# zhaobinglei/REGNet_for_3D_Grasping

Hardware: AMD Instinct MI355X
Metric: scenes/sec (25 600-pt ScoreNet+GRN fwd) (higher is better)
Workload: dtype f32; 1 GPU; configs[2]: ScoreNet+GraspRegionNet+RefineNet forward, 25600-pt synthetic scenes, batch=8 per GPU, eval; points=25600, batch_per_gpu=8, global_batch=8, parallelism=scene-sharded x1 (no data-path collective), sampling_group_batches=8, sampling_lookahead_batches=32, distinct_batches=8, region_head=synthetic.calibrate_region_head on batch 0, geometry_pending_at_enqueue=4, hip_graphs=False

## Files before the change

### include/regnet_hip.h

```cpp
#ifndef REGNET_HIP_H_
#define REGNET_HIP_H_

#include <stdint.h>

#ifdef __cplusplus
extern "C" {
#endif

#define REGNET_OK 0
#define REGNET_ERR_SHAPE (-1)
#define REGNET_ERR_NULL (-2)
#define REGNET_ERR_UNSUPPORTED (-3)

int regnet_abi_version(void);
const char* regnet_build_info(void);
const char* regnet_strerror(int code);

int regnet_fps_f32(const float* xyz, int64_t sb, int64_t sc, int64_t sn, int64_t B, int64_t N,
                   int64_t M, int64_t* index, float* workspace, void* stream);
int64_t regnet_fps_workspace_bytes(int64_t B, int64_t N, int64_t M);
int regnet_fps_chain_f32(const float* xyz, int64_t sb, int64_t sc, int64_t sn, int64_t B, int64_t N, int64_t M,
                         int64_t* index, float* workspace, const int32_t* prefix_ok, int32_t* first_tie, void* stream);
int64_t regnet_fps_status_offset_bytes(int64_t B, int64_t N, int64_t M);
int regnet_fps_plan(int64_t B, int64_t N, int64_t M, int64_t* plan);
// ... 179 lines not shown
                                int64_t label_ld, int64_t C, float radius, float score_thre, int64_t m, float* final_grasp,
                                uint8_t* flags, float* terms, float* dreg, void* stream);

int regnet_gripper_frame_f32(const float* grasp, int64_t ld, int64_t n, float* centre, float* rot, void* stream);
int regnet_crop_pick(const int32_t* cand, int64_t G, const int64_t* pos, int64_t R, const uint8_t* valid,
                     const int64_t* group_index, int64_t gi_stride, int64_t n, int64_t* index, int64_t* index_inall,
                     void* stream);

int regnet_resample_groups_f32(const float* pc, int64_t pb, int64_t pn, int64_t C, const int32_t* cand, int64_t cap,
                               const int64_t* pos, int64_t B, int64_t Nc, int64_t G, int64_t N, int32_t* out_of_range,
                               int64_t* index, float* points, void* stream);

int64_t regnet_normals_workspace_bytes(int64_t N);
int regnet_estimate_normals_f32(const float* xyz, int64_t N, double radius, int64_t max_nn, double cam_x, double cam_y,
                                double cam_z, float* normals, int32_t* count, void* workspace, void* stream);

int64_t regnet_bn_workspace_bytes(int64_t C);
int regnet_bn_relu_train_fwd_f32(const float* x, int64_t B, int64_t C, int64_t L, const float* gamma, const float* beta,
                                 float eps, float momentum, float* running_mean, float* running_var, int relu,
                                 int64_t pool_group, float* y, int32_t* pool_index, float* save_mean, float* save_invstd,
                                 void* workspace, void* stream);
int regnet_bn_relu_train_bwd_f32(const float* x, const float* y, const float* dy, const int32_t* pool_index, int64_t B,
                                 int64_t C, int64_t L, const float* gamma, const float* beta, const float* save_mean,
                                 const float* save_invstd, int relu, int64_t pool_group, float* dx, float* dgamma,
                                 float* dbeta, void* workspace, void* stream);

int regnet_bn_train_stats_f32(const float* x, int64_t B, int64_t C, int64_t L, const float* gamma, const float* beta, float eps,
                              float momentum, float* running_mean, float* running_var, float* save_mean, float* save_invstd,
                              float* scale, float* shift, void* workspace, void* stream);
int regnet_bn_relu_train_fwd_from_sums_f32(const float* x, int64_t B, int64_t C, int64_t L, const float* gamma, const float* beta,
                                           float eps, float momentum, float* running_mean, float* running_var, int relu,
                                           int64_t pool_group, float* y, int32_t* pool_index, float* save_mean,
                                           float* save_invstd, void* workspace, void* stream);
int regnet_bn_train_stats_from_sums_f32(int64_t B, int64_t C, int64_t L, const float* gamma, const float* beta, float eps,
                                        float momentum, float* running_mean, float* running_var, float* save_mean,
                                        float* save_invstd, float* scale, float* shift, void* workspace, void* stream);

int regnet_sa_premul_layer_f32(const float* U, int64_t ldu, const float* V, int64_t ldv, int64_t C1,
                               const int64_t* nbr, int64_t B, int64_t Nsrc, int64_t M, int64_t group,
                               const float* W, int64_t Kpad, const float* scale, const float* shift,
                               float* C, int64_t ldc, int64_t N, int relu, int pool_group, void* stream);

int regnet_interp_concat_f32(const float* sparse, int64_t sb, int64_t sn, int64_t Cs,
                             const int64_t* idx, const float* dist2, float eps, const float* dense,
                             int64_t db, int64_t dn, int64_t dc, int64_t Cd, int64_t B, int64_t Nd,
                             float* out, int64_t ldo, int64_t Cout, void* stream);

int regnet_interp_affine_f32(const float* ys, int64_t sb, int64_t sn, const int64_t* idx,
                             const float* dist2, float eps, const float* yd, int64_t ldd,
                             const float* dense_small, int64_t db, int64_t dn, int64_t dc,
                             int64_t Cd_small, const float* Wd4, const float* scale, const float* shift,
                             int relu, int64_t B, int64_t Nd, int64_t C, float* out, int64_t ldo,
                             void* stream);

int regnet_score_head_f32(const float* x, int64_t ldx, int64_t C, const float* w, float bias,
                          float bn_scale, float bn_shift, float* score, int64_t P, void* stream);

int64_t regnet_sa_premul_chain_stream_floats(void);
int regnet_sa_premul_chain_f32(const float* U, int64_t ldu, const float* V, int64_t ldv, const int64_t* nbr, int64_t B,
                               int64_t Nsrc, int64_t M, const float* stream_w, int64_t n_stages, const float* affine,
                               int64_t affine_floats, int relu3, float* out, int64_t ldo, int32_t* ticket,
                               void* stream);

int64_t regnet_sa3_premul_chain_stream_floats(void);
int regnet_sa3_premul_chain_f32(const float* U, int64_t ldu, const float* V, int64_t ldv, const int64_t* nbr, int64_t B,
                                int64_t Nsrc, int64_t M, const float* stream_w, int64_t n_stages, const float* affine,
                                int64_t affine_floats, int relu3, float* out, int64_t ldo, int32_t* ticket,
                                void* stream);

int64_t regnet_fp_head_chain_stream_floats(void);
int64_t regnet_fp_head_chain_blocks(int64_t P);
int regnet_fp_head_chain_interp_f32(const float* Ys, int64_t ys_sb, int64_t ys_sn, const int64_t* idx,
                                    const float* dist2, float eps, const float* dense_small, int64_t db, int64_t dn,
                                    int64_t dc, int64_t Cd_small, const float* tables, int64_t B, int64_t Nd,
                                    const float* stream_w, int64_t n_stages, const float* affine, int64_t affine_floats,
                                    const float* wscore, float score_bias, float score_bn_scale, float score_bn_shift,
                                    float* F, int64_t ldf, float* score, int32_t* ticket, int64_t block_first,
                                    int64_t block_count, void* stream);
int regnet_fp_head_chain_f32(const float* X, int64_t ldx, const float* stream_w, int64_t n_stages,
                             const float* affine, int64_t affine_floats, const float* wscore, float score_bias,
                             float score_bn_scale, float score_bn_shift, float* F, int64_t ldf, float* score,
                             int64_t P, int32_t* ticket, int64_t block_first, int64_t block_count, void* stream);

int regnet_conv1x1_train_supported(int64_t Co, int64_t Ci, int64_t L);
int regnet_conv1x1_fwd_f32(const float* W, const float* X, float* Y, int64_t B, int64_t Co, int64_t Ci, int64_t L,
                           void* stream);
int regnet_conv1x1_dgrad_f32(const float* W, const float* dY, float* dX, int64_t B, int64_t Co, int64_t Ci, int64_t L,
                             void* stream);
int regnet_conv1x1_fwd_stream_f32(const float* W, const float* X, float* Y, int64_t B, int64_t Co, int64_t Ci, int64_t L,
                                  int32_t* ticket, void* stream);
int regnet_conv1x1_dgrad_stream_f32(const float* W, const float* dY, float* dX, int64_t B, int64_t Co, int64_t Ci, int64_t L,
                                    int32_t* ticket, void* stream);
int regnet_conv1x1_fwd_smallci_f32(const float* W, const float* X, float* Y, int64_t B, int64_t Co, int64_t Ci, int64_t L,
                                   void* stream);
int64_t regnet_conv1x1_smallci_stats_workspace_bytes(int64_t B, int64_t Ci, int64_t L);
int regnet_conv1x1_fwd_smallci_stats_f32(const float* W, const float* X, float* Y, int64_t B, int64_t Co, int64_t Ci, int64_t L,
                                         void* workspace, void* sums, void* stream);
int64_t regnet_conv1x1_wgrad_smallci_partials(int64_t B, int64_t Co, int64_t L);
int regnet_conv1x1_wgrad_smallci_f32(const float* dY, const float* X, float* part, int64_t B, int64_t Co, int64_t Ci, int64_t L,
                                     void* stream);
int regnet_conv1x1_smallco_f32(int dir, const float* W, const float* bias, const float* in, float* out, int64_t B, int64_t Co,
                               int64_t Ci, int64_t L, void* stream);
int regnet_conv1x1_stream_reserve_slots(int slots);
int64_t regnet_sa_chain3_split_plane_bytes(int64_t C3);
int regnet_sa_chain3_split_f32(const float* feat, int64_t fb, int64_t fn, int64_t fc, int64_t Cf, const float* xyz, int64_t xb,
                               int64_t xc, int64_t xn, const int64_t* nbr, const int64_t* ctr, const int64_t* count,
// ... 86 lines not shown
```

### regnet_for_3d_grasping_amd/csrc/gemm2.h

```cpp
#pragma once
#include "common.h"

typedef float g2_f32x16 __attribute__((ext_vector_type(16)));

#define G2_BK 16

struct G2Args {
  const float* A; long long lda; int Ka;
  const float* W; int Kpad;
  const float* scale; const float* shift;
  float* C; long long ldc;
  long long P; int N; int relu;
  int tiles_m, tiles_n;
  int main_blocks, tail_tiles, tail_split;
};

__device__ __forceinline__ void g2_glds16(const float* gsrc, unsigned lds_dst) {
  unsigned keep;
  asm volatile("s_mov_b32 %0, m0\n\ts_mov_b32 m0, %2\n\ts_nop 0\n\tglobal_load_lds_dwordx4 %1, off\n\ts_mov_b32 m0, %0"
               : "=&s"(keep) : "v"(gsrc), "s"(lds_dst) : "memory");
}

template <int N> __device__ __forceinline__ void g2_wait_barrier() {
  asm volatile("s_waitcnt vmcnt(%0)\n\ts_barrier" :: "i"(N) : "memory");
}

__device__ __forceinline__ long long g2_xcd_linear(unsigned vblock, long long total) {
  const long long q = total / 8, r = total % 8;
  const long long xcd = vblock % 8, s = vblock / 8;
  return (xcd < r ? xcd * (q + 1) : r * (q + 1) + (xcd - r) * q) + s;
}

template <int ROWS_MAX, int TBN, int WM, int WN, int TM, int STAGES, bool POOL, int SLAB_KT>
__device__ __forceinline__ void g2_tile(const G2Args& p, float* smem, long long row0, int col0) {
  constexpr int NW = WM * WN;
  constexpr int ROWS = WM * TM * 32;
  constexpr int TN = TBN / WN / 32;
  constexpr int STAGE_FLOATS = (ROWS_MAX + TBN) * G2_BK;
  constexpr int GROUPS = (ROWS + TBN) / 16;
  constexpr int L = (GROUPS + NW - 1) / NW;
  static_assert(GROUPS % NW == 0, "every wave issues the same number of LDS-DMA pieces");
  constexpr int D = STAGES - 1;
  const int tid = threadIdx.x, lane = tid & 63;
  const int wave = __builtin_amdgcn_readfirstlane(tid >> 6);
  const int wm = wave / WN, wn = wave % WN;
  const int fr = lane & 31, fh = lane >> 5;

  const float* gp[L];
  unsigned dst[L];
  bool isA[L];
  const int lrow = lane >> 2, lchunk = (lane & 3) ^ ((lane >> 4) & 3);
#pragma unroll
  for (int j = 0; j < L; ++j) {
    const int grp = wave + j * NW;
    const int cr = grp * 16 + lrow;
    isA[j] = grp * 16 < ROWS;
    if (isA[j]) {
      long long r = row0 + cr;
      if (r >= p.P) r = 0;
      gp[j] = p.A + r * p.lda + 4 * lchunk;
    } else {
      gp[j] = p.W + (long long)(col0 + cr - ROWS) * p.Kpad + 4 * lchunk;
    }
    dst[j] = (unsigned)(grp * 16 * G2_BK * 4);
  }
  const unsigned smem_base = (unsigned)(uintptr_t)smem;
  const bool ragged_k = p.Ka < p.Kpad;

#define G2_ISSUE(KT_, STAGE_)                                                                                   \
  _Pragma("unroll") for (int j = 0; j < L; ++j) {                                                                \
    const float* src = gp[j] + (long long)(KT_) * G2_BK;                                                         \
    if (ragged_k && isA[j] && (KT_) * G2_BK + 4 * lchunk >= p.Ka) src = gp[j] - 4 * lchunk;    \
    g2_glds16(src, smem_base + (unsigned)((STAGE_) * STAGE_FLOATS * 4) + dst[j]);                                \
  }

  g2_f32x16 acc[TM][TN];
#pragma unroll
  for (int mi = 0; mi < TM; ++mi)
#pragma unroll
    for (int ni = 0; ni < TN; ++ni)
#pragma unroll
      for (int r = 0; r < 16; ++r) acc[mi][ni][r] = 0.f;

  g2_f32x16 tot[SLAB_KT > 0 ? TM : 1][SLAB_KT > 0 ? TN : 1];
  if constexpr (SLAB_KT > 0) {
#pragma unroll
// ... 33 lines not shown
#define G2_PIN() __builtin_amdgcn_sched_barrier(0)
#else
#define G2_PIN()
#endif
#define G2_COMPUTE(STAGE_)                                                                                        \
  {                                                                                                               \
    const float* st = smem + (STAGE_) * STAGE_FLOATS;                                                             \
    float4 a[2][TM], b[2][TN];        \
    _Pragma("unroll") for (int kk = 0; kk < 2; ++kk) {                                                            \
      _Pragma("unroll") for (int mi = 0; mi < TM; ++mi)                                                           \
        a[kk][mi] = *reinterpret_cast<const float4*>(st + offA[kk] + mi * 32 * G2_BK);                            \
      _Pragma("unroll") for (int ni = 0; ni < TN; ++ni)                                                           \
        b[kk][ni] = *reinterpret_cast<const float4*>(st + offW[kk] + ni * 32 * G2_BK);                            \
    }                                                                                                             \
    G2_PIN();                                                                                                     \
    _Pragma("unroll") for (int kk = 0; kk < 2; ++kk)                                                              \
      _Pragma("unroll") for (int mi = 0; mi < TM; ++mi)                                                           \
        _Pragma("unroll") for (int ni = 0; ni < TN; ++ni) {                                                       \
          acc[mi][ni] = __builtin_amdgcn_mfma_f32_32x32x2f32(a[kk][mi].x, b[kk][ni].x, acc[mi][ni], 0, 0, 0);     \
          acc[mi][ni] = __builtin_amdgcn_mfma_f32_32x32x2f32(a[kk][mi].y, b[kk][ni].y, acc[mi][ni], 0, 0, 0);     \
          acc[mi][ni] = __builtin_amdgcn_mfma_f32_32x32x2f32(a[kk][mi].z, b[kk][ni].z, acc[mi][ni], 0, 0, 0);     \
          acc[mi][ni] = __builtin_amdgcn_mfma_f32_32x32x2f32(a[kk][mi].w, b[kk][ni].w, acc[mi][ni], 0, 0, 0);     \
        }                                                                                                         \
  }
#pragma unroll
  for (int d = 0; d < D; ++d) { G2_ISSUE(d, d) }
  int stage = 0;
  for (int kt = 0; kt < KT - D; ++kt) {
    g2_wait_barrier<(D - 1) * L>();
    int ns = stage + D; if (ns >= STAGES) ns -= STAGES;
    G2_ISSUE(kt + D, ns)
    G2_COMPUTE(stage)
    G2_SLAB()
    if (++stage == STAGES) stage = 0;
  }
#pragma unroll
  for (int d = 0; d < D; ++d) {
    g2_wait_barrier<0>();
    G2_COMPUTE(stage)
    G2_SLAB()
    if (++stage == STAGES) stage = 0;
  }
  if constexpr (SLAB_KT > 0) {
#pragma unroll
    for (int mi = 0; mi < TM; ++mi)
#pragma unroll
      for (int ni = 0; ni < TN; ++ni)
#pragma unroll
        for (int r = 0; r < 16; ++r) acc[mi][ni][r] += tot[mi][ni][r];
  }
#undef G2_SLAB
#undef G2_COMPUTE
#undef G2_ISSUE
#pragma unroll
  for (int ni = 0; ni < TN; ++ni) {
    const int col = col0 + (wn * TN + ni) * 32 + fr;
    const bool col_ok = col < p.N;
    const float s = col_ok ? p.scale[col] : 0.f, t = col_ok ? p.shift[col] : 0.f;
    if (POOL) {
      static_assert(!POOL || TM == 2, "pooling: a wave's 64 rows are one neighbourhood");
      float m = -__builtin_inff();
#pragma unroll
      for (int mi = 0; mi < TM; ++mi)
#pragma unroll
        for (int r = 0; r < 16; ++r) {
          float y = acc[mi][ni][r] * s + t;
          if (p.relu) y = fmaxf(y, 0.f);
          m = fmaxf(m, y);
        }
      m = fmaxf(m, __shfl_xor(m, 32, 64));
      const long long wrow = row0 + wm * 64;
      if (col_ok && fh == 0 && wrow < p.P) p.C[(wrow / 64) * p.ldc + col] = m;
    } else {
      const long long first_row = row0 + wm * TM * 32 + 4 * fh;
      float* cp = p.C + first_row * p.ldc + col;
      const long long ld = p.ldc;
      const bool interior = (row0 + ROWS <= p.P) && (col0 + TBN <= p.N);
      if (interior) {
#pragma unroll
        for (int mi = 0; mi < TM; ++mi)
#pragma unroll
          for (int r = 0; r < 16; ++r) {
            float y = acc[mi][ni][r] * s + t;
            if (p.relu) y = fmaxf(y, 0.f);
            *cp = y;
            cp += ((r & 3) == 3) ? 5 * ld : ld;
          }
      } else {
#pragma unroll
        for (int mi = 0; mi < TM; ++mi)
#pragma unroll
          for (int r = 0; r < 16; ++r) {
            float y = acc[mi][ni][r] * s + t;
            if (p.relu) y = fmaxf(y, 0.f);
            if (col_ok && first_row + mi * 32 + (r & 3) + 8 * (r >> 2) < p.P) *cp = y;
            cp += ((r & 3) == 3) ? 5 * ld : ld;
          }
      }
    }
  }
}

#ifndef G2_SLAB_KT
#define G2_SLAB_KT 8
#endif
template <int TBM, int TBN, int WM, int WN, int WG_PER_CU> struct G2Slab {
  static constexpr int acc_tiles = (TBM / WM / 32) * (TBN / WN / 32);
  static constexpr int kt = (acc_tiles <= 2 || (acc_tiles <= 4 && WG_PER_CU * WM * WN <= 8)) ? G2_SLAB_KT : 0;
};

template <int TBM, int TBN, int WM, int WN, int STAGES, int WG_PER_CU, bool POOL>
__global__ __launch_bounds__(WM * WN * 64, WG_PER_CU * WM * WN / 4)
void gemm2_kernel(const G2Args p) {
  constexpr int SLAB = G2Slab<TBM, TBN, WM, WN, WG_PER_CU>::kt;
  constexpr int TM = TBM / WM / 32;
  __shared__ __attribute__((aligned(1024))) float smem[STAGES * (TBM + TBN) * G2_BK];
  const int bid = blockIdx.x;
  if (bid < p.main_blocks) {
    const long long t = g2_xcd_linear((unsigned)bid, p.main_blocks);
    const int tm = (int)(t / p.tiles_n), tn = (int)(t % p.tiles_n);
    g2_tile<TBM, TBN, WM, WN, TM, STAGES, POOL, SLAB>(p, smem, (long long)tm * TBM, tn * TBN);
  } else if constexpr (!POOL && TM == 2 && ((WM * 32 + TBN) / 16) % (WM * WN) == 0) {
    const int t = (bid - p.main_blocks) / p.tail_split, s = (bid - p.main_blocks) % p.tail_split;
    const long long tile = (long long)p.main_blocks + t;
    const int tm = (int)(tile / p.tiles_n), tn = (int)(tile % p.tiles_n);
    g2_tile<TBM, TBN, WM, WN, 1, STAGES, false, SLAB>(p, smem, (long long)tm * TBM + (long long)s * (TBM / 2), tn * TBN);
  }
}
```

### regnet_for_3d_grasping_amd/csrc/mlp.hip

```cpp
#include <stdlib.h>
#include "common.h"
#include "gemm2.h"

typedef float f32x16 __attribute__((ext_vector_type(16)));

#define BM 128
#define BN 128
#define MLP_THREADS 256
#ifndef MLP_BK
#define MLP_BK 16
#endif
#define BK MLP_BK
#ifndef MLP_ABLATE
#define MLP_ABLATE 0
#endif
#ifndef MLP_TRACE
#define MLP_TRACE 0
#endif
#define LDS_LD (BK + 4)
#define ROWS_PER_PASS (MLP_THREADS / (BK / 4))
#define STAGE_PASSES (BM / ROWS_PER_PASS)
#ifndef MLP_MIN_WAVES
#define MLP_MIN_WAVES (BK == 32 ? 2 : 4)
#endif
// ... 403 lines not shown
};

template <int TBM, int TBN, int WM, int WN, int STAGES, int OCC>
static int plan_gemm2_tile(int tile, long long P, int N, bool pool, G2Plan& pl) {
  pl.tile = tile; pl.tbm = TBM; pl.tbn = TBN; pl.waves = WM * WN; pl.wg_per_cu = OCC;
  pl.slab_kt = G2Slab<TBM, TBN, WM, WN, OCC>::kt;
  pl.tiles_m = (int)((P + TBM - 1) / TBM);
  pl.tiles_n = (N + TBN - 1) / TBN;
  const long long tiles = (long long)pl.tiles_m * pl.tiles_n;
  if (tiles >= (1ll << 30)) return REGNET_ERR_UNSUPPORTED;
  const long long slots = (long long)G2_CUS * OCC;
  long long main_blocks = tiles, tail_tiles = 0;
  constexpr bool can_split = (TBM / WM / 32 == 2) && ((WM * 32 + TBN) / 16) % (WM * WN) == 0;
  if (!pool && can_split && tiles > slots) {
    const long long rem = tiles % slots;
    if (rem > 0 && rem * 2 <= slots) { main_blocks = tiles - rem; tail_tiles = rem; }
  }
  pl.main_blocks = (int)main_blocks; pl.tail_tiles = (int)tail_tiles; pl.tail_split = 2;
  if (pool && TBM / WM != 64) return REGNET_ERR_UNSUPPORTED;
  return REGNET_OK;
}

static int plan_gemm2(long long P, int N, int Kpad, bool pool, G2Plan& pl) {
  static const int force_tile = getenv("REGNET_G2_TILE") ? atoi(getenv("REGNET_G2_TILE")) : -1;
  if (force_tile == 0) return plan_gemm2_tile<G2_TILE_256>(0, P, N, pool, pl);
  if (force_tile == 1) return plan_gemm2_tile<G2_TILE_128>(1, P, N, pool, pl);
  if (force_tile == 2) return plan_gemm2_tile<G2_TILE_64>(2, P, N, pool, pl);
  if (force_tile == 3 && !pool) return plan_gemm2_tile<G2_TILE_128W8>(3, P, N, pool, pl);
  if (force_tile == 8 && !pool) return plan_gemm2_tile<G2_TILE_128S>(8, P, N, pool, pl);
  const long long nt = (N + 127) / 128;
  const long long t256 = ((P + 255) / 256) * nt, t128 = ((P + 127) / 128) * nt;
  if (N > 128 && t256 >= 4 * G2_CUS) return plan_gemm2_tile<G2_TILE_256>(0, P, N, pool, pl);
  static const bool t8 = !(getenv("REGNET_G2_T8") && getenv("REGNET_G2_T8")[0] == '0');
  if (t8 && !pool && G2_SLAB_KT > 0 && Kpad >= 2 * G2_SLAB_KT * G2_BK && t128 >= G2_CUS)
    return plan_gemm2_tile<G2_TILE_128S>(8, P, N, pool, pl);
  if (t128 >= 4 * G2_CUS && (G2_SLAB_KT == 0 || Kpad < 2 * G2_SLAB_KT * G2_BK || pool))
    return plan_gemm2_tile<G2_TILE_128>(1, P, N, pool, pl);
  return plan_gemm2_tile<G2_TILE_64>(2, P, N, pool, pl);
}

template <int TBM, int TBN, int WM, int WN, int STAGES, int OCC>
static int launch_gemm2_tile(const G2Args& g, bool pool, hipStream_t st) {
  const dim3 grid((unsigned)(g.main_blocks + g.tail_split * g.tail_tiles)), block(WM * WN * 64);
  if (pool) {
    if constexpr (TBM / WM == 64) hipLaunchKernelGGL((gemm2_kernel<TBM, TBN, WM, WN, STAGES, OCC, true>), grid, block, 0, st, g);
    else return REGNET_ERR_UNSUPPORTED;
  } else {
    hipLaunchKernelGGL((gemm2_kernel<TBM, TBN, WM, WN, STAGES, OCC, false>), grid, block, 0, st, g);
  }
  REGNET_LAUNCH_CHECK();
  return REGNET_OK;
}

static int launch_gemm2(G2Args g, const G2Plan& pl, bool pool, hipStream_t st) {
  g.tiles_m = pl.tiles_m; g.tiles_n = pl.tiles_n;
  g.main_blocks = pl.main_blocks; g.tail_tiles = pl.tail_tiles; g.tail_split = pl.tail_split;
  switch (pl.tile) {
    case 0: return launch_gemm2_tile<G2_TILE_256>(g, pool, st);
    case 1: return launch_gemm2_tile<G2_TILE_128>(g, pool, st);
    case 2: return launch_gemm2_tile<G2_TILE_64>(g, pool, st);
    case 3: return launch_gemm2_tile<G2_TILE_128W8>(g, pool, st);
    case 8: return launch_gemm2_tile<G2_TILE_128S>(g, pool, st);
  }
  return REGNET_ERR_UNSUPPORTED;
}

struct MlpLayerPlan { bool gemm2; G2Plan g2; long long blocks; };
static int plan_mlp_layer(long long P, long long N, long long Kpad, int pool_group, MlpLayerPlan& pl) {
  pl = MlpLayerPlan{};
  if (P < 0 || N <= 0 || Kpad <= 0 || Kpad % BK) return REGNET_ERR_SHAPE;
  if (pool_group != 0 && (pool_group != 64 || P % 64)) return REGNET_ERR_UNSUPPORTED;
  if (P == 0) return REGNET_OK;
  static const bool use_gemm2 = MLP_USE_GEMM2 && !(getenv("REGNET_GEMM2") && getenv("REGNET_GEMM2")[0] == '0');
  if (use_gemm2 && Kpad >= 2 * G2_BK) {
    pl.gemm2 = true;
    return plan_gemm2(P, (int)N, (int)Kpad, pool_group != 0, pl.g2);
  }
  pl.blocks = ((P + BM - 1) / BM) * ((N + BN - 1) / BN);
  return pl.blocks >= (1ll << 31) ? REGNET_ERR_UNSUPPORTED : REGNET_OK;
}

extern "C" int regnet_mlp_layer_plan(int64_t P, int64_t N, int64_t Kpad, int pool_group, int64_t* plan) {
  if (!plan) return REGNET_ERR_NULL;
  for (int i = 0; i < 8; ++i) plan[i] = 0;
  MlpLayerPlan pl;
  const int rc = plan_mlp_layer(P, N, Kpad, pool_group, pl);
  if (rc != REGNET_OK || P == 0) return rc;
  if (pl.gemm2) {
    const G2Plan& g = pl.g2;
    plan[0] = g.tbm; plan[1] = g.tbn; plan[2] = g.waves; plan[3] = g.wg_per_cu; plan[4] = g.slab_kt;
    plan[5] = g.main_blocks; plan[6] = g.tail_tiles; plan[7] = g.tail_tiles ? g.tail_split : 0;
  } else {
    plan[5] = pl.blocks;
  }
  return REGNET_OK;
}

extern "C" int regnet_mlp_layer_f32(const float* A, int64_t lda, int64_t Ka, const float* W, int64_t Kpad,
                                    const float* scale, const float* shift, float* C, int64_t ldc, int64_t P,
                                    int64_t N, int relu, int pool_group, void* stream) {
  if (P < 0 || N <= 0 || Ka < 0 || Kpad <= 0 || Kpad % BK || Ka > Kpad || (Ka & 3) || (lda & 3)) return REGNET_ERR_SHAPE;
  if (pool_group != 0 && (pool_group != 64 || P % 64)) return REGNET_ERR_UNSUPPORTED;
  if (P == 0) return REGNET_OK;
  if (!A || !W || !scale || !shift || !C) return REGNET_ERR_NULL;
  if (!aligned16(A) || !aligned16(W)) return REGNET_ERR_SHAPE;
  MlpLayerPlan pl;
  const int rc = plan_mlp_layer(P, N, Kpad, pool_group, pl);
  if (rc != REGNET_OK) return rc;
  if (pl.gemm2) {
    G2Args g = {};
    g.A = A; g.lda = lda; g.Ka = (int)Ka; g.W = W; g.Kpad = (int)Kpad; g.scale = scale; g.shift = shift;
    g.C = C; g.ldc = ldc; g.P = P; g.N = (int)N; g.relu = relu;
    return launch_gemm2(g, pl.g2, pool_group != 0, as_stream(stream));
  }
  MlpArgs a = {};
  a.A = A; a.lda = lda; a.Ka = (int)Ka;
  a.W = W; a.Kpad = (int)Kpad; a.scale = scale; a.shift = shift;
  a.C = C; a.ldc = ldc; a.P = P; a.N = (int)N; a.relu = relu; a.group = 64; a.rows_per_scene = 1;
  return launch_gemm(a, 0, pool_group != 0, as_stream(stream));
}

__global__ __launch_bounds__(256) void splitk_finish_kernel(const float* __restrict__ part, int S, long long P, int N,
                                                            long long ldp, const float* __restrict__ scale,
                                                            const float* __restrict__ shift, int relu,
                                                            float* __restrict__ C, long long ldc) {
  const long long i = (long long)blockIdx.x * 256 + threadIdx.x;
  if (i >= P * N) return;
  const long long row = i / N;
  const int col = (int)(i - row * N);
  float acc = part[row * ldp + col];
  for (int s = 1; s < S; ++s) acc += part[(long long)s * P * ldp + row * ldp + col];
  float y = acc * scale[col] + shift[col];
  if (relu) y = fmaxf(y, 0.f);
  C[row * ldc + col] = y;
}

extern "C" int64_t regnet_mlp_splitk_workspace_bytes(int64_t P, int64_t N, int64_t ksplit) {
  return ksplit > 1 ? ksplit * P * ((N + 3) / 4 * 4) * (int64_t)sizeof(float) : 0;
}

extern "C" int regnet_mlp_layer_splitk_f32(const float* A, int64_t lda, int64_t Ka, const float* W, int64_t Kpad,
                                           const float* scale, const float* shift, float* C, int64_t ldc, int64_t P,
                                           int64_t N, int relu, int64_t ksplit, void* workspace, void* stream) {
  if (P < 0 || N <= 0 || Ka < 0 || Kpad <= 0 || Kpad % BK || Ka > Kpad || (Ka & 3) || (lda & 3) || ksplit < 1)
    return REGNET_ERR_SHAPE;
  if (ksplit > Kpad / BK || P * N >= (1ll << 40)) return REGNET_ERR_UNSUPPORTED;
  if (P == 0) return REGNET_OK;
  if (!A || !W || !scale || !shift || !C || (ksplit > 1 && !workspace)) return REGNET_ERR_NULL;
  if (!aligned16(A) || !aligned16(W) || (ksplit > 1 && !aligned16(workspace))) return REGNET_ERR_SHAPE;
  MlpArgs a = {};
  a.A = A; a.lda = lda; a.Ka = (int)Ka;
  a.W = W; a.Kpad = (int)Kpad; a.scale = scale; a.shift = shift;
  a.P = P; a.N = (int)N; a.relu = relu; a.group = 64; a.rows_per_scene = 1;
  if (ksplit == 1) {
    a.C = C; a.ldc = ldc;
    return launch_gemm(a, 0, false, as_stream(stream));
  }
  const long long ldp = (N + 3) / 4 * 4;
  a.C = (float*)workspace; a.ldc = ldp; a.ksplit = (int)ksplit;
  int rc = launch_gemm(a, 0, false, as_stream(stream));
  if (rc) return rc;
  const long long blocks = (P * N + 255) / 256;
  if (blocks >= (1ll << 31)) return REGNET_ERR_UNSUPPORTED;
  hipLaunchKernelGGL(splitk_finish_kernel, dim3((unsigned)blocks), dim3(256), 0, as_stream(stream),
                     (const float*)workspace, (int)ksplit, (long long)P, (int)N, ldp, scale, shift, relu, C,
                     (long long)ldc);
  REGNET_LAUNCH_CHECK();
  return REGNET_OK;
}

extern "C" int regnet_sa_layer1_f32(const float* feat, int64_t fb, int64_t fn, int64_t fc, int64_t Cf,
                                    const float* xyz, int64_t xb, int64_t xc, int64_t xn, const int64_t* nbr,
// ... 225 lines not shown
```

### regnet_for_3d_grasping_amd/fused.py

```python
import torch

from . import _lib, pn2_ext

ENABLED = True
CHAIN3 = True
SPLITK_MAX_ROWS = 1024
PREMUL = True
PREMUL_CENTRE = True

_call = _lib.call
_L = _lib.lib


def _f32_weights(module):
    p = next(module.parameters(), None)
    return p is None or p.dtype == torch.float32


def usable(module, xyz):
    return (ENABLED and xyz.is_cuda and xyz.dtype == torch.float32 and not module.training and not torch.is_grad_enabled()
            and _f32_weights(module))


def supports_sa(module, feature):
# ... 285 lines not shown
          l2.W.data_ptr(), l2.Kpad, l2.scale.data_ptr(), l2.shift.data_ptr(), l2.N,
          l3.W.data_ptr(), l3.Kpad, l3.scale.data_ptr(), l3.shift.data_ptr(), l3.N, l3.relu, out.data_ptr(), out.stride(0))
    return out


def interp_concat(sparse_cl, idx, dist2, eps, dense_feature, B, Nd):
    Cs = sparse_cl.size(2)
    Cd = 0 if dense_feature is None else dense_feature.size(1)
    width = _round_up(Cs + Cd, 4)
    out = torch.empty((B * Nd, width), dtype=torch.float32, device=sparse_cl.device)
    dptr, db, dc, dn, _ = _strided3(dense_feature)
    _call("regnet_interp_concat_f32", sparse_cl, sparse_cl.data_ptr(), sparse_cl.stride(0), sparse_cl.stride(1), Cs,
          idx.data_ptr(), dist2.data_ptr(), float(eps), dptr, db, dn, dc, Cd, B, Nd, out.data_ptr(), out.stride(0), width)
    return out, width


def _fp_split_layers(first, Cs):
    def part(cols):
        K, Kpad = cols.shape[1], _round_up(max(cols.shape[1], 1), 16)
        Wp = torch.zeros((first.W.shape[0], Kpad), dtype=torch.float32, device=first.W.device)
        Wp[:, :K] = cols
        return _Layer(W=Wp.contiguous(), scale=torch.ones_like(first.scale), shift=torch.zeros_like(first.shift), N=first.N,
                      K=K, Kpad=Kpad, relu=0)

    def build():
        Cd = first.K - Cs
        wd4 = None
        if 0 < Cd <= 4:
            wd4 = torch.zeros((first.N, 4), dtype=torch.float32, device=first.W.device)
            wd4[:, :Cd] = first.W[:first.N, Cs:first.K]
            wd4 = wd4.contiguous()
        return part(first.W[:, :Cs]), part(first.W[:, Cs:first.K]) if Cd > 4 else None, wd4
    return _derived(first, "fp_split", build)


def _interp_tables(first, wd4):
    def build():
        wd = wd4 if wd4 is not None else torch.zeros((256, 4), dtype=torch.float32, device=first.W.device)
        return torch.cat([wd.reshape(-1), first.scale[:256], first.shift[:256]]).contiguous()
    return _derived(first, "interp_tables", build)


def interp_affine(Ys, idx, dist2, eps, Yd, dense_small, wd4, layer, B, Ns, Nd):
    C = layer.N
    out = torch.empty((B * Nd, C), dtype=torch.float32, device=Ys.device)
    dptr, db, dc, dn, Cd = _strided3(dense_small)
    wptr = None if dense_small is None else wd4.data_ptr()
    _call("regnet_interp_affine_f32", Ys, Ys.data_ptr(), Ns * Ys.stride(0), Ys.stride(0), idx.data_ptr(), dist2.data_ptr(),
          float(eps), None if Yd is None else Yd.data_ptr(), 0 if Yd is None else Yd.stride(0), dptr, db, dn, dc, Cd, wptr,
          layer.scale.data_ptr(), layer.shift.data_ptr(), layer.relu, B, Nd, C, out.data_ptr(), out.stride(0))
    return out


def _packed_head(seg):
    def build():
        conv, bn = seg.conv_score, seg.bn_score
        w = conv.weight.detach().reshape(-1).float().contiguous()
        bn_scale = float(bn.weight.detach()[0] / torch.sqrt(bn.running_var.detach()[0] + bn.eps))
        bn_shift = float(bn.bias.detach()[0] - bn.running_mean.detach()[0] * bn_scale)
        bias = float(conv.bias.detach()[0]) if conv.bias is not None else 0.0
        return w, bias, bn_scale, bn_shift
    return _cached(seg, "score_head", _signature(seg.conv_score) + _signature(seg.bn_score), build)


def score_head(x, seg, P):
    w, bias, bn_scale, bn_shift = _packed_head(seg)
    score = torch.empty((P,), dtype=torch.float32, device=x.device)
    _call("regnet_score_head_f32", x, x.data_ptr(), x.stride(0), w.numel(), w.data_ptr(), bias, bn_scale, bn_shift,
          score.data_ptr(), P)
    return score


def _flop_meta(P, K, N):
    return "P%d K%d N%d flop%d" % (P, K, N, 2 * P * K * N)


TIMED_OPS = {
    "mlp_layer": lambda A, Ka, layer, P, pool_group=0: _flop_meta(P, layer.K, layer.N) + (" pool%d" % pool_group if pool_group else ""),
    "sa_layer1": lambda feature, xyz, nbr, ctr, layer, B, M, group: _flop_meta(B * M * group, layer.K, layer.N),
    "sa_premul_layer": lambda U, V, nbr, layer, B, Nsrc, M, group, pool_group=0:
        _flop_meta(B * M * group, layer.K, layer.N),
    "sa_chain3": lambda feature, xyz, nbr, ctr, l1, l2, l3, B, M, group, count=None, order=None:
        "P%d K%d N%d flop%d" % (B * M * group, l3.K, l3.N,
                                2 * B * M * group * (l1.K * l1.N + l2.K * l2.N + l3.K * l3.N)),
    "sa_premul_chain": lambda U, V, nbr, module, layers, B, Nsrc, M:
        "P%d K256 N512 flop%d" % (B * M * 64, 2 * B * M * 64 * (256 * 256 + 256 * 512)),
    "sa3_premul_chain": lambda U, V, nbr, module, layers, B, Nsrc, M:
        "P%d K512 N1024 flop%d" % (B * M * 64, 2 * B * M * 64 * (512 * 512 + 512 * 1024)),
    "fp_head_chain_interp": lambda Ys, idx, dist2, eps, dense_small, wd4, first, seg, fp_layers, B, Ns, Nd:
        "P%d K256 N256 flop%d" % (B * Nd, 2 * B * Nd * 491520),
    "fp_head_chain": lambda h1, seg, fp_layers, P: "P%d K256 N256 flop%d" % (P, 2 * P * 491520),
    "sa_layer12": lambda feature, xyz, nbr, ctr, first, layer, B, M, group, pool_group=0:
        "P%d K%d N%d flop%d" % (B * M * group, layer.K, layer.N,
                                2 * B * M * group * (layer.K * layer.N + first.K * first.N)),
}


def _as_channels_last(feature):
    cl = feature.transpose(1, 2)
    return cl if cl.is_contiguous() else cl.contiguous()


def sa_sample(module, xyz, prefix_ok=None):
    chain = pn2_ext.FpsChain(prefix_ok if FPS_CHAIN else None)
    ctr = pn2_ext.farthest_point_sample(xyz, module.num_centroids, chain)
    return ctr, chain.first_tie


def sa_group(module, xyz, ctr, first_tie=None):
    B, M = ctr.shape
    new_xyz = pn2_ext.gather_points(xyz, ctr) if xyz.dtype == torch.float32 else torch.gather(xyz, 2, ctr[:, None, :].expand(B, 3, M))
    nbr, count = pn2_ext.ball_query(xyz, new_xyz, module.grouper.radius, module.grouper.num_neighbours)
    geo = {"ctr": ctr, "new_xyz": new_xyz, "nbr": nbr}
    if first_tie is not None:
        geo["first_tie"] = first_tie
    if (CHAIN3 and module.grouper.num_neighbours == 64 and len(module.mlp) == 3
            and module.mlp[0].conv.in_channels <= 8):
        geo["count"] = count
        geo["order"] = chain3_pair_order(count)
    elif (PREMUL and not module.training and not torch.is_grad_enabled() and module.use_xyz
          and module.mlp[0].conv.in_channels > 8 and len(module.mlp) >= 2):
        Cf = module.mlp[0].conv.in_channels - 3
        layers = _packed_stack(module, module.mlp,
                               lambda: torch.cat([torch.arange(3, 3 + Cf), torch.arange(0, 3)]).to(xyz.device))
        first = layers[0]
        if first.relu and first.N % 4 == 0 and layers[1].K == first.N:
            _, v_layer = _premul_layers(first, Cf)
            geo["mu"] = xyz.mean(dim=2, keepdim=True) if PREMUL_CENTRE else None
            geo["V"] = mlp_layer(pack_rows(None, new_xyz, 4, geo["mu"]), 4, v_layer, B * M)
            geo["V_layer"] = v_layer
    return geo
# ... 30 lines not shown
        rest = layers[2:]
    elif PREMUL and feature is not None and layers[0].relu and layers[0].N % 4 == 0 and layers[1].K == layers[0].N:
        first, N1 = layers[0], xyz.shape[2]
        u_layer, v_layer = _premul_layers(first, Cf)
        width = _round_up(Cf + 3, 4)
        if "V" in geo and geo.get("V_layer") is v_layer:
            mu, V = geo["mu"], geo["V"]
        elif "V" in geo:
            mu = geo["mu"]
            V = mlp_layer(pack_rows(None, geo["new_xyz"], 4, mu), 4, v_layer, B * M)
        else:
            mu = xyz.mean(dim=2, keepdim=True) if PREMUL_CENTRE else None
            V = mlp_layer(pack_rows(None, geo["new_xyz"], 4, mu), 4, v_layer, B * M)
        U = mlp_layer(pack_rows(feature, xyz, width, mu), width, u_layer, B * N1)
        if supports_sa3_chain(layers) and U.size(1) == 512:
            pooled = sa3_premul_chain(U, V, geo["nbr"], module, layers, B, N1, M)
            return geo["new_xyz"], pooled.view(B, M, -1).transpose(1, 2)
        if supports_sa_chain(layers) and U.size(1) == 256:
            pooled = sa_premul_chain(U, V, geo["nbr"], module, layers, B, N1, M)
            return geo["new_xyz"], pooled.view(B, M, -1).transpose(1, 2)
        if len(layers) == 2:
            pooled = sa_premul_layer(U, V, geo["nbr"], layers[1], B, N1, M, K, pool_group=K)
            return geo["new_xyz"], pooled.view(B, M, -1).transpose(1, 2)
        h = sa_premul_layer(U, V, geo["nbr"], layers[1], B, N1, M, K)
        rest = layers[2:]
    else:
        h = sa_layer1(feature, xyz, geo["nbr"], geo["ctr"], layers[0], B, M, K)
        rest = layers[1:]
    for layer in rest[:-1]:
        h = mlp_layer(h, layer.K, layer, P)
    pooled = mlp_layer(h, rest[-1].K, rest[-1], P, pool_group=K)
    return geo["new_xyz"], pooled.view(B, M, -1).transpose(1, 2)


def sa_forward(module, xyz, feature, geo=None):
    return sa_features(module, xyz, feature, geo if geo is not None else sa_geometry(module, xyz))


def fp_geometry(module, dense_xyz, sparse_xyz):
    idx, dist2 = pn2_ext.point_search(dense_xyz, sparse_xyz, module.interpolator.num_neighbors)
    return {"idx": idx, "dist2": dist2}


def _fp_first_layer(module, layers, dense_xyz, dense_feature, sparse_feature, geo):
    B, _, Nd = dense_xyz.shape
    Cs, Ns = sparse_feature.size(1), sparse_feature.size(2)
    Cd = 0 if dense_feature is None else dense_feature.size(1)
    first = layers[0]
    if not (PREMUL and first.N % 4 == 0 and 256 % (first.N // 4) == 0 and Cs % 4 == 0 and (Cd % 4 == 0 or Cd <= 4)
            and Ns < Nd and first.K == Cs + Cd and (dense_feature is None or dense_feature.dtype == torch.float32)):
        return None
    lay_s, lay_d, wd4 = _fp_split_layers(first, Cs)
    Ys = mlp_layer(_as_channels_last(sparse_feature).view(B * Ns, Cs), Cs, lay_s, B * Ns)
    Yd = None
    if lay_d is not None:
        Yd = mlp_layer(_as_channels_last(dense_feature).view(B * Nd, Cd), Cd, lay_d, B * Nd)
    return interp_affine(Ys, geo["idx"], geo["dist2"], module.interpolator._eps, Yd,
                         dense_feature if wd4 is not None else None, wd4, first, B, Ns, Nd)


def fp_features(module, dense_xyz, dense_feature, sparse_feature, geo):
    B, _, Nd = dense_xyz.shape
    layers = _packed_stack(module, module.mlp)
    h = _fp_first_layer(module, layers, dense_xyz, dense_feature, sparse_feature, geo)
    if h is not None:
        Ka, layers = layers[0].N, layers[1:]
    else:
        h, Ka = interp_concat(_as_channels_last(sparse_feature), geo["idx"], geo["dist2"], module.interpolator._eps,
                              dense_feature, B, Nd)
    for layer in layers:
        h = mlp_layer(h, Ka, layer, B * Nd)
        Ka = layer.N
    return h.view(B, Nd, -1).transpose(1, 2)


def fp_forward(module, dense_xyz, sparse_xyz, dense_feature, sparse_feature, geo=None):
    if geo is None:
        geo = fp_geometry(module, dense_xyz, sparse_xyz)
    return fp_features(module, dense_xyz, dense_feature, sparse_feature, geo)


def head_forward(seg, sparse_feature):
    B, C, N = sparse_feature.shape
    layers = _packed_stack(seg.mlp, seg.mlp)
    h = _as_channels_last(sparse_feature).view(B * N, C)
    Ka = C
    if Ka % 4:
        raise NotImplementedError("head input width must be a multiple of 4")
    for layer in layers:
        h = mlp_layer(h, Ka, layer, B * N)
        Ka = layer.N
    return score_head(h, seg, B * N).view(B, N)


def _packed_premul_chain(module, layers, C):
    def build():
        l2, l3 = layers[1], layers[2]
        halves = range(C // 256)
        stages = [_swizzle_stage(l2.W[32 * rg:32 * rg + 32, 256 * kh:256 * kh + 256]) for kh in halves for rg in range(C // 32)]
        stages += [_swizzle_stage(l3.W[32 * s:32 * s + 32, 256 * kh:256 * kh + 256]) for s in range(C // 16) for kh in halves]
        stream = torch.cat(stages).contiguous()
        affine = torch.cat([l2.scale[:C], l2.shift[:C], l3.scale[:2 * C], l3.shift[:2 * C]]).contiguous()
        floats = _L.regnet_sa_premul_chain_stream_floats() if C == 256 else _L.regnet_sa3_premul_chain_stream_floats()
        assert stream.numel() == floats and affine.numel() == 6 * C
        return stream, affine
    return _cached(module, "sa_chain" if C == 256 else "sa3_chain", _signature(module.mlp), build)


def _premul_chain(C, U, V, nbr, module, layers, B, Nsrc, M):
    stream, affine = _packed_premul_chain(module, layers, C)
# ... 323 lines not shown
```

Baseline: 1063 scenes/s.

## Fuse three-NN interpolation and BN affine into the dense-skip GEMM epilogue

For feature-propagation first layers that have a dense skip input, the dense-projection GEMM now does the three-neighbour inverse-distance interpolation of the sparse projection in its epilogue, adds it to the accumulator and applies scale, shift and ReLU before storing. This removes the intermediate Yd tensor write and read, plus the separate interp_affine kernel launch. The epilogue loads per-row weights and offsets into LDS and gathers three Ys rows per output element, which adds scattered loads and register pressure inside the GEMM tile. If the plan is not gemm2, it falls back to the old path.

```diff
diff --git a/include/regnet_hip.h b/include/regnet_hip.h
--- a/include/regnet_hip.h
+++ b/include/regnet_hip.h
@@ -255,6 +255,11 @@
                              int64_t Cd_small, const float* Wd4, const float* scale, const float* shift,
                              int relu, int64_t B, int64_t Nd, int64_t C, float* out, int64_t ldo,
                              void* stream);
+
+int regnet_mlp_layer_interp_f32(const float* A, int64_t lda, int64_t Ka, const float* W, int64_t Kpad,
+                                const float* ys, int64_t ldy, const int64_t* idx, const float* dist2, float eps,
+                                const float* scale, const float* shift, int relu, int64_t B, int64_t Ns,
+                                int64_t Nd, int64_t N, float* C, int64_t ldc, void* stream);
 
 int regnet_score_head_f32(const float* x, int64_t ldx, int64_t C, const float* w, float bias,
                           float bn_scale, float bn_shift, float* score, int64_t P, void* stream);
diff --git a/regnet_for_3d_grasping_amd/csrc/gemm2.h b/regnet_for_3d_grasping_amd/csrc/gemm2.h
--- a/regnet_for_3d_grasping_amd/csrc/gemm2.h
+++ b/regnet_for_3d_grasping_amd/csrc/gemm2.h
@@ -13,7 +13,19 @@
   long long P; int N; int relu;
   int tiles_m, tiles_n;
   int main_blocks, tail_tiles, tail_split;
+  const float* ys; unsigned ldy;
+  const long long* idx; const float* dist2; float eps;
+  unsigned Nd, Ns;
 };
+
+__device__ __forceinline__ float g2_interp_value(float a0, float a1, float a2, float w0, float w1, float w2, float d, float sc,
+                                                 float sh, int relu) {
+  float v = __builtin_fmaf(a2, w2, __builtin_fmaf(a0, w0, a1 * w1));
+  v = v + d;
+  v = __builtin_fmaf(v, sc, sh);
+  if (relu) v = fmaxf(v, 0.f);
+  return v;
+}
 
 __device__ __forceinline__ void g2_glds16(const float* gsrc, unsigned lds_dst) {
   unsigned keep;
@@ -31,7 +43,7 @@
   return (xcd < r ? xcd * (q + 1) : r * (q + 1) + (xcd - r) * q) + s;
 }
 
-template <int ROWS_MAX, int TBN, int WM, int WN, int TM, int STAGES, bool POOL, int SLAB_KT>
+template <int ROWS_MAX, int TBN, int WM, int WN, int TM, int STAGES, bool POOL, int SLAB_KT, bool INTERP = false>
 __device__ __forceinline__ void g2_tile(const G2Args& p, float* smem, long long row0, int col0) {
   constexpr int NW = WM * WN;
   constexpr int ROWS = WM * TM * 32;
@@ -171,6 +183,62 @@
 #undef G2_SLAB
 #undef G2_COMPUTE
 #undef G2_ISSUE
+  if constexpr (INTERP) {
+    static_assert(!INTERP || !POOL, "the interpolating epilogue stores every row");
+    static_assert(6 * ROWS <= STAGES * STAGE_FLOATS, "row tables fit the ring");
+    __syncthreads();
+    float* wgt = smem;
+    unsigned* yoff = reinterpret_cast<unsigned*>(smem + 3 * ROWS);
+    for (int rt = tid; rt < ROWS; rt += NW * 64) {
+      long long pr = row0 + rt;
+      if (pr >= p.P) pr = 0;
+      const unsigned b = (unsigned)pr / p.Nd;
+      const float i0 = 1.0f / fmaxf(p.dist2[pr * 3], p.eps), i1 = 1.0f / fmaxf(p.dist2[pr * 3 + 1], p.eps),
+                  i2 = 1.0f / fmaxf(p.dist2[pr * 3 + 2], p.eps);
+      const float norm = (i0 + i1) + i2;
+      wgt[rt] = i0 / norm; wgt[ROWS + rt] = i1 / norm; wgt[2 * ROWS + rt] = i2 / norm;
+#pragma unroll
+      for (int k = 0; k < 3; ++k) {
+        long long j = p.idx[pr * 3 + k];
+        j = j < 0 ? 0 : (j >= (long long)p.Ns ? (long long)p.Ns - 1 : j);
+        yoff[k * ROWS + rt] = (b * p.Ns + (unsigned)j) * p.ldy;
+      }
+    }
+    __syncthreads();
+    float s[TN], t[TN];
+    int colv[TN];
+    bool col_okv[TN];
+#pragma unroll
+    for (int ni = 0; ni < TN; ++ni) {
+      const int col = col0 + (wn * TN + ni) * 32 + fr;
+      col_okv[ni] = col < p.N;
+      colv[ni] = col_okv[ni] ? col : 0;
+      s[ni] = p.scale[colv[ni]]; t[ni] = p.shift[colv[ni]];
+    }
+    const int rt0 = wm * TM * 32 + 4 * fh;
+    const long long ld = p.ldc;
+    float* cp = p.C + (row0 + rt0) * ld + (col0 + wn * TN * 32 + fr);
+    const bool interior = (row0 + ROWS <= p.P) && (col0 + TBN <= p.N);
+#define G2_INTERP_ROWS(GUARD_)                                                                                    \
+    _Pragma("unroll") for (int mi = 0; mi < TM; ++mi)                                                             \
+      _Pragma("unroll") for (int r = 0; r < 16; ++r) {                                                            \
+        const int rt = rt0 + mi * 32 + (r & 3) + 8 * (r >> 2);                                                    \
+        const float w0 = wgt[rt], w1 = wgt[ROWS + rt], w2 = wgt[2 * ROWS + rt];                                   \
+        const float* y0 = p.ys + yoff[rt];                                                                        \
+        const float* y1 = p.ys + yoff[ROWS + rt];                                                                 \
+        const float* y2 = p.ys + yoff[2 * ROWS + rt];                                                             \
+        const bool row_ok = !(GUARD_) || row0 + rt < p.P;                                                         \
+        _Pragma("unroll") for (int ni = 0; ni < TN; ++ni) {                                                       \
+          const float y = g2_interp_value(y0[colv[ni]], y1[colv[ni]], y2[colv[ni]], w0, w1, w2, acc[mi][ni][r],   \
+                                          s[ni], t[ni], p.relu);                                                  \
+          if (row_ok && (!(GUARD_) || col_okv[ni])) cp[ni * 32] = y;                                              \
+        }                                                                                                         \
+        cp += ((r & 3) == 3) ? 5 * ld : ld;                                                                       \
+      }
+    if (interior) { G2_INTERP_ROWS(false) } else { G2_INTERP_ROWS(true) }
+#undef G2_INTERP_ROWS
+    return;
+  }
 #pragma unroll
   for (int ni = 0; ni < TN; ++ni) {
     const int col = col0 + (wn * TN + ni) * 32 + fr;
@@ -228,7 +296,7 @@
   static constexpr int kt = (acc_tiles <= 2 || (acc_tiles <= 4 && WG_PER_CU * WM * WN <= 8)) ? G2_SLAB_KT : 0;
 };
 
-template <int TBM, int TBN, int WM, int WN, int STAGES, int WG_PER_CU, bool POOL>
+template <int TBM, int TBN, int WM, int WN, int STAGES, int WG_PER_CU, bool POOL, bool INTERP = false>
 __global__ __launch_bounds__(WM * WN * 64, WG_PER_CU * WM * WN / 4)
 void gemm2_kernel(const G2Args p) {
   constexpr int SLAB = G2Slab<TBM, TBN, WM, WN, WG_PER_CU>::kt;
@@ -238,11 +306,11 @@
   if (bid < p.main_blocks) {
     const long long t = g2_xcd_linear((unsigned)bid, p.main_blocks);
     const int tm = (int)(t / p.tiles_n), tn = (int)(t % p.tiles_n);
-    g2_tile<TBM, TBN, WM, WN, TM, STAGES, POOL, SLAB>(p, smem, (long long)tm * TBM, tn * TBN);
+    g2_tile<TBM, TBN, WM, WN, TM, STAGES, POOL, SLAB, INTERP>(p, smem, (long long)tm * TBM, tn * TBN);
   } else if constexpr (!POOL && TM == 2 && ((WM * 32 + TBN) / 16) % (WM * WN) == 0) {
     const int t = (bid - p.main_blocks) / p.tail_split, s = (bid - p.main_blocks) % p.tail_split;
     const long long tile = (long long)p.main_blocks + t;
     const int tm = (int)(tile / p.tiles_n), tn = (int)(tile % p.tiles_n);
-    g2_tile<TBM, TBN, WM, WN, 1, STAGES, false, SLAB>(p, smem, (long long)tm * TBM + (long long)s * (TBM / 2), tn * TBN);
-  }
-}
+    g2_tile<TBM, TBN, WM, WN, 1, STAGES, false, SLAB, INTERP>(p, smem, (long long)tm * TBM + (long long)s * (TBM / 2), tn * TBN);
+  }
+}
diff --git a/regnet_for_3d_grasping_amd/csrc/mlp.hip b/regnet_for_3d_grasping_amd/csrc/mlp.hip
--- a/regnet_for_3d_grasping_amd/csrc/mlp.hip
+++ b/regnet_for_3d_grasping_amd/csrc/mlp.hip
@@ -479,6 +479,27 @@
   return REGNET_OK;
 }
 
+template <int TBM, int TBN, int WM, int WN, int STAGES, int OCC>
+static int launch_gemm2_interp_tile(const G2Args& g, hipStream_t st) {
+  const dim3 grid((unsigned)(g.main_blocks + g.tail_split * g.tail_tiles)), block(WM * WN * 64);
+  hipLaunchKernelGGL((gemm2_kernel<TBM, TBN, WM, WN, STAGES, OCC, false, true>), grid, block, 0, st, g);
+  REGNET_LAUNCH_CHECK();
+  return REGNET_OK;
+}
+
+static int launch_gemm2_interp(G2Args g, const G2Plan& pl, hipStream_t st) {
+  g.tiles_m = pl.tiles_m; g.tiles_n = pl.tiles_n;
+  g.main_blocks = pl.main_blocks; g.tail_tiles = pl.tail_tiles; g.tail_split = pl.tail_split;
+  switch (pl.tile) {
+    case 0: return launch_gemm2_interp_tile<G2_TILE_256>(g, st);
+    case 1: return launch_gemm2_interp_tile<G2_TILE_128>(g, st);
+    case 2: return launch_gemm2_interp_tile<G2_TILE_64>(g, st);
+    case 3: return launch_gemm2_interp_tile<G2_TILE_128W8>(g, st);
+    case 8: return launch_gemm2_interp_tile<G2_TILE_128S>(g, st);
+  }
+  return REGNET_ERR_UNSUPPORTED;
+}
+
 static int launch_gemm2(G2Args g, const G2Plan& pl, bool pool, hipStream_t st) {
   g.tiles_m = pl.tiles_m; g.tiles_n = pl.tiles_n;
   g.main_blocks = pl.main_blocks; g.tail_tiles = pl.tail_tiles; g.tail_split = pl.tail_split;
@@ -545,6 +566,32 @@
   a.W = W; a.Kpad = (int)Kpad; a.scale = scale; a.shift = shift;
   a.C = C; a.ldc = ldc; a.P = P; a.N = (int)N; a.relu = relu; a.group = 64; a.rows_per_scene = 1;
   return launch_gemm(a, 0, pool_group != 0, as_stream(stream));
+}
+
+extern "C" int regnet_mlp_layer_interp_f32(const float* A, int64_t lda, int64_t Ka, const float* W, int64_t Kpad,
+                                           const float* ys, int64_t ldy, const int64_t* idx, const float* dist2, float eps,
+                                           const float* scale, const float* shift, int relu, int64_t B, int64_t Ns,
+                                           int64_t Nd, int64_t N, float* C, int64_t ldc, void* stream) {
+  if (B < 0 || Nd < 0 || Ns <= 0 || N <= 0 || Ka < 0 || Kpad <= 0 || Kpad % BK || Ka > Kpad || (Ka & 3) || (lda & 3) ||
+      ldy < N || ldc < N)
+    return REGNET_ERR_SHAPE;
+  if (B > (1ll << 31) / (Nd > 0 ? Nd : 1) || B * Nd >= (1ll << 31) || ldy >= (1ll << 31) || B > (1ll << 31) / Ns ||
+      B * Ns > ((1ll << 31) - 1) / ldy)
+    return REGNET_ERR_UNSUPPORTED;
+  const long long P = B * Nd;
+  if (P == 0) return REGNET_OK;
+  if (!A || !W || !ys || !idx || !dist2 || !scale || !shift || !C) return REGNET_ERR_NULL;
+  if (!aligned16(A) || !aligned16(W)) return REGNET_ERR_SHAPE;
+  MlpLayerPlan pl;
+  const int rc = plan_mlp_layer(P, N, Kpad, 0, pl);
+  if (rc != REGNET_OK) return rc;
+  if (!pl.gemm2) return REGNET_ERR_UNSUPPORTED;
+  G2Args g = {};
+  g.A = A; g.lda = lda; g.Ka = (int)Ka; g.W = W; g.Kpad = (int)Kpad; g.scale = scale; g.shift = shift;
+  g.C = C; g.ldc = ldc; g.P = P; g.N = (int)N; g.relu = relu;
+  g.ys = ys; g.ldy = (unsigned)ldy; g.idx = (const long long*)idx; g.dist2 = dist2; g.eps = eps;
+  g.Nd = (unsigned)Nd; g.Ns = (unsigned)Ns;
+  return launch_gemm2_interp(g, pl.g2, as_stream(stream));
 }
 
 __global__ __launch_bounds__(256) void splitk_finish_kernel(const float* __restrict__ part, int S, long long P, int N,
diff --git a/regnet_for_3d_grasping_amd/fused.py b/regnet_for_3d_grasping_amd/fused.py
--- a/regnet_for_3d_grasping_amd/fused.py
+++ b/regnet_for_3d_grasping_amd/fused.py
@@ -361,6 +361,27 @@
     return out
 
 
+_UNSUPPORTED = -3
+FP_EPILOGUE_INTERP = True
+
+
+def mlp_layer_interp(A, Ka, lay_d, Ys, idx, dist2, eps, layer, B, Ns, Nd):
+    out = torch.empty((B * Nd, layer.N), dtype=torch.float32, device=A.device)
+    rc = _call("regnet_mlp_layer_interp_f32", A, A.data_ptr(), A.stride(0), Ka, lay_d.W.data_ptr(), lay_d.Kpad, Ys.data_ptr(),
+               Ys.stride(0), idx.data_ptr(), dist2.data_ptr(), float(eps), layer.scale.data_ptr(), layer.shift.data_ptr(),
+               layer.relu, B, Ns, Nd, layer.N, out.data_ptr(), out.stride(0), tolerate=_UNSUPPORTED)
+    return None if rc == _UNSUPPORTED else out
+
+
+def fp_skip_interp(Ys, dense_cl, Cd, lay_d, first, idx, dist2, eps, B, Ns, Nd):
+    if FP_EPILOGUE_INTERP:
+        h = mlp_layer_interp(dense_cl, Cd, lay_d, Ys, idx, dist2, eps, first, B, Ns, Nd)
+        if h is not None:
+            return h
+    Yd = mlp_layer(dense_cl, Cd, lay_d, B * Nd)
+    return interp_affine(Ys, idx, dist2, eps, Yd, None, None, first, B, Ns, Nd)
+
+
 def _packed_head(seg):
     def build():
         conv, bn = seg.conv_score, seg.bn_score
@@ -386,6 +407,7 @@
 
 TIMED_OPS = {
     "mlp_layer": lambda A, Ka, layer, P, pool_group=0: _flop_meta(P, layer.K, layer.N) + (" pool%d" % pool_group if pool_group else ""),
+    "mlp_layer_interp": lambda A, Ka, lay_d, Ys, idx, dist2, eps, layer, B, Ns, Nd: _flop_meta(B * Nd, lay_d.K, lay_d.N),
     "sa_layer1": lambda feature, xyz, nbr, ctr, layer, B, M, group: _flop_meta(B * M * group, layer.K, layer.N),
     "sa_premul_layer": lambda U, V, nbr, layer, B, Nsrc, M, group, pool_group=0:
         _flop_meta(B * M * group, layer.K, layer.N),
@@ -522,10 +544,10 @@
         return None
     lay_s, lay_d, wd4 = _fp_split_layers(first, Cs)
     Ys = mlp_layer(_as_channels_last(sparse_feature).view(B * Ns, Cs), Cs, lay_s, B * Ns)
-    Yd = None
     if lay_d is not None:
-        Yd = mlp_layer(_as_channels_last(dense_feature).view(B * Nd, Cd), Cd, lay_d, B * Nd)
-    return interp_affine(Ys, geo["idx"], geo["dist2"], module.interpolator._eps, Yd,
+        return fp_skip_interp(Ys, _as_channels_last(dense_feature).view(B * Nd, Cd), Cd, lay_d, first, geo["idx"],
+                              geo["dist2"], module.interpolator._eps, B, Ns, Nd)
+    return interp_affine(Ys, geo["idx"], geo["dist2"], module.interpolator._eps, None,
                          dense_feature if wd4 is not None else None, wd4, first, B, Ns, Nd)
 
 
```

Result: no change. 1070 scenes/s (median of 6 runs) (+0.7%).
